# pangenome/impg

Hardware: AMD Instinct MI355X
Metric: projected ranges/sec, 1M-PAF 100k-BED -x depth 3; CPU coitrees baseline (higher is better)
Workload: dtype int32

## Files before the change

impg_amd/_lib.py:

```python
import ctypes as C
import os
import subprocess

import numpy as np

_HERE = os.path.dirname(os.path.abspath(__file__))
LIB_PATH = os.environ.get("IMPG_GPU_LIB") or os.path.join(_HERE, "libimpg_gpu.so")
CSRC = os.path.join(_HERE, "csrc")

IMPG_OK = 0
IMPG_E_INVALID, IMPG_E_HIP, IMPG_E_OOM, IMPG_E_IO, IMPG_E_UNSUPPORTED, IMPG_E_CANCELLED = -1, -2, -3, -4, -5, -6
STREAM_CB = C.CFUNCTYPE(C.c_int, C.c_void_p, C.c_void_p, C.c_size_t)
ORDER_COITREES, ORDER_SORTED = 0, 1
HIT_NONE = 0xFFFFFFFF

RECORD_DTYPE = np.dtype([("query_id", "<u4"), ("target_id", "<u4"), ("query_start", "<i4"), ("query_end", "<i4"),
                         ("target_start", "<i4"), ("target_end", "<i4"), ("cigar_off", "<u8"), ("cigar_len", "<u4"),
                         ("strand", "<u4")], align=True)
RANGE_DTYPE = np.dtype([("target_id", "<u4"), ("start", "<i4"), ("end", "<i4")])
INTERVAL_DTYPE = np.dtype([("query_id", "<u4"), ("q_first", "<i4"), ("q_last", "<i4"),
                           ("target_id", "<u4"), ("t_first", "<i4"), ("t_last", "<i4")])
assert RECORD_DTYPE.itemsize == 40 and RANGE_DTYPE.itemsize == 12
TP_RECORD_DTYPE = np.dtype([("query_id", "<u4"), ("target_id", "<u4"), ("query_start", "<i4"), ("query_end", "<i4"),
                            ("target_start", "<i4"), ("target_end", "<i4"), ("seg_off", "<u8"), ("n_segs", "<u4"),
# ... 96 lines not shown
    ("impg_gpu_query_batch_filtered", C.c_int, [_P, _P, C.c_size_t, C.POINTER(Params), _P, _P, C.POINTER(_P)]),
    ("impg_gpu_parse_subsequence", C.c_int, [C.c_char_p, C.c_char_p, C.c_size_t, C.POINTER(C.c_int32)]),
    ("impg_gpu_subset_keep", C.c_int, [C.c_char_p, C.c_size_t, _P, C.c_size_t, _P, C.POINTER(C.c_size_t)]),
    ("impg_gpu_query", C.c_int, [_P, C.c_uint32, C.c_int32, C.c_int32, C.POINTER(Params), C.POINTER(_P)]),
    ("impg_gpu_results_num_ranges", C.c_size_t, [_P]),
    ("impg_gpu_results_total", C.c_size_t, [_P]),
    ("impg_gpu_results_offsets", _P, [_P]),
    ("impg_gpu_results_intervals", _P, [_P]),
    ("impg_gpu_results_projected", C.c_uint64, [_P]),
    ("impg_gpu_results_cigar_offsets", _P, [_P]),
    ("impg_gpu_results_cigar_ops", _P, [_P]),
    ("impg_gpu_results_timing", None, [_P, C.POINTER(C.c_double), C.POINTER(C.c_double)]),
    ("impg_gpu_results_free", None, [_P]),
    ("impg_gpu_query_batch_stats", C.c_int, [_P, _P, C.c_size_t, C.POINTER(Params), _P, _P, C.POINTER(Stats)]),
    ("impg_gpu_query_batch_stats_dev", C.c_int, [_P, _P, C.c_size_t, C.POINTER(Params), _P, _P, C.POINTER(Stats)]),
    ("impg_gpu_query_batch_device", C.c_int, [_P, _P, C.c_size_t, C.c_int, C.POINTER(Params), C.c_int, C.POINTER(_P)]),
    ("impg_gpu_device_rows_num_parts", C.c_size_t, [_P]),
    ("impg_gpu_device_rows_part", C.c_int, [_P, C.c_size_t, C.POINTER(DevicePart)]),
    ("impg_gpu_device_rows_stats", None, [_P, C.POINTER(Stats)]),
    ("impg_gpu_device_rows_place_ms", C.c_float, [_P]),
    ("impg_gpu_device_rows_part_device", C.c_int, [_P, C.c_size_t, C.POINTER(C.c_int)]),
    ("impg_gpu_device_rows_batch_offset", C.c_int, [_P, C.POINTER(C.c_uint64), C.POINTER(C.c_uint64)]),
    ("impg_gpu_device_rows_check", C.c_int, [_P, _P, _P]),
    ("impg_gpu_device_rows_free", None, [_P]),
    ("impg_gpu_bed_merge", C.c_long, [_P, C.c_size_t, C.c_int32, C.c_int]),
    ("impg_gpu_results_bed", C.c_int, [_P, _P, _P, C.POINTER(Params), C.c_int32, C.POINTER(_P), C.POINTER(C.c_size_t)]),
    ("impg_gpu_query_batch_bed", C.c_int, [_P, _P, C.c_size_t, C.POINTER(Params), _P, C.c_int32, _P, C.POINTER(_P), C.POINTER(C.c_size_t),
                                           _P]),
    ("impg_gpu_query_batch_bed_fd", C.c_int, [_P, _P, C.c_size_t, C.POINTER(Params), _P, C.c_int32, _P, C.c_int, C.POINTER(C.c_uint64), _P]),
    ("impg_gpu_results_paf", C.c_int, [_P, _P, _P, C.POINTER(Params), C.c_int32, C.c_int, C.POINTER(_P), C.POINTER(C.c_size_t)]),
    ("impg_gpu_parse_cigar", C.c_long, [C.c_char_p, C.c_size_t, _P, C.c_size_t]),
    ("impg_gpu_parse_target_range", C.c_int, [C.c_char_p, C.c_char_p, C.c_size_t, C.POINTER(C.c_int32), C.POINTER(C.c_int32)]),
    ("impg_gpu_comm_unique_id", C.c_int, [_P, C.c_int]),
    ("impg_gpu_comm_create_rccl", C.c_int, [_P, C.c_int, C.c_int, C.c_int, C.c_int, C.POINTER(_P)]),
    ("impg_gpu_comm_create_host", C.c_int, [_P, C.c_int, C.c_int, C.c_int, C.c_int, C.POINTER(_P)]),
    ("impg_gpu_comm_destroy", None, [_P]),
    ("impg_gpu_comm_info", C.c_int, [_P, C.POINTER(C.c_int), C.POINTER(C.c_int), C.POINTER(C.c_int), C.POINTER(C.c_char_p)]),
    ("impg_gpu_comm_check", C.c_int, [_P, C.c_int]),
    ("impg_gpu_index_create_rank", C.c_int, [_P, C.c_size_t, _P, C.c_size_t, _P, C.c_uint32, _P, C.c_uint32, C.c_int, C.c_int,
                                             C.c_int, _P, C.POINTER(_P)]),
    ("impg_gpu_index_create_from_paf_rank", C.c_int, [C.POINTER(C.c_char_p), C.c_int, C.c_int, C.c_int, C.c_int, _P, C.POINTER(_P)]),
    ("impg_gpu_index_create_multi", C.c_int, [_P, C.c_size_t, _P, C.c_size_t, _P, C.c_uint32, _P, C.c_uint32, C.c_int, C.c_int,
                                              _P, C.c_int, C.c_int, C.POINTER(_P)]),
    ("impg_gpu_index_create_from_paf_multi", C.c_int, [C.POINTER(C.c_char_p), C.c_int, C.c_int, C.c_int, _P, C.c_int, C.c_int,
                                                       C.POINTER(_P)]),
    ("impg_gpu_shard_assign", C.c_int, [_P, C.c_uint32, C.c_uint32, _P]),
    ("impg_gpu_index_shard_info", C.c_int, [_P, C.POINTER(C.c_int), C.POINTER(C.c_int), C.POINTER(C.c_int), _P, C.c_size_t]),
    ("impg_gpu_index_hop_profile", C.c_int, [_P, _P, C.c_size_t, C.c_int, C.POINTER(C.c_size_t)]),
    ("impg_synth_paf", C.c_int, [C.c_uint64, C.c_size_t, C.c_uint32, C.c_int32, C.c_int32, C.c_uint32, _P, _P, C.c_size_t,
                                 C.POINTER(C.c_size_t)]),
    ("impg_synth_paf_text", C.c_int, [C.c_uint64, C.c_size_t, C.c_uint32, C.c_int32, C.c_int32, C.c_uint32, C.c_char_p]),
    ("impg_synth_skewed_paf_text", C.c_int, [C.c_uint64, C.c_size_t, C.c_uint32, C.c_int32, C.c_char_p, C.POINTER(C.c_uint64)]),
    ("impg_gpu_selftest_order_sort", C.c_int, [C.c_int, C.c_uint32, C.c_uint, C.c_uint64]),
    ("impg_synth_seq_name", C.c_int, [C.c_uint32, C.c_char_p, C.c_size_t]),
    ("impg_synth_bed", C.c_int, [C.c_uint64, C.c_size_t, C.c_uint32, C.c_int32, C.c_int32, _P]),
]

_LIB = None


def lib():
    global _LIB
    if _LIB is None:
        if not os.path.exists(LIB_PATH):
            raise RuntimeError("libimpg_gpu.so is not built: run `python -c 'import __graft_entry__ as g; g.build()'` "
                               "or `make -C impg_amd/csrc` (there is no CPU fallback)")
        L = C.CDLL(LIB_PATH)
        for name, res, args in SYMBOLS:
            f = getattr(L, name)
            f.restype = res
            f.argtypes = args
        _LIB = L
    return _LIB


def check(rc):
    if rc != IMPG_OK:
        raise ImpgGpuError(rc, lib().impg_gpu_last_error().decode(errors="replace"))


def free(ptr):
    C.CDLL(None).free(ptr)
```

impg_amd/csrc/capi.cpp:

```cpp
#include <sys/stat.h>
#include <unistd.h>

#include <atomic>
#include <cerrno>
#include <functional>
#include <thread>
#include <chrono>
#include <cmath>
#include <cstdlib>
#include <memory>
#include <new>

#include "engine.hpp"

namespace impg {
thread_local std::string g_error;
void set_error(const std::string &msg) { g_error = msg; }
void render_paf(const impg_gpu_results &res, const impg_gpu_index &ix, const char *const *range_names,
                const impg_gpu_params_t &p, int32_t merge_distance, bool bedpe, std::vector<std::string> &parts);
void render_bed(const impg_gpu_results &res, const impg_gpu_index &ix, const char *const *range_names,
                const impg_gpu_params_t &p, int32_t merge_distance, std::vector<std::string> &parts);
char *join_parts(std::vector<std::string> &parts, size_t *len);
}

// ... 1218 lines not shown
  std::vector<std::string> parts;
  render_paf(*res, *ix, range_names, *params, merge_distance, format == IMPG_OUT_BEDPE, parts);
  *text = join_parts(parts, len);
  return IMPG_OK;
  IMPG_CATCH
}

int impg_gpu_selftest_order_sort(int device, uint32_t n, unsigned end_bit, uint64_t seed) {
  IMPG_TRY
  if (end_bit < 1 || end_bit > 32) throw Error{IMPG_E_INVALID, "end_bit is 1 .. 32"};
  IMPG_HIP(hipSetDevice(device));
  std::vector<uint32_t> keys(n), perm(n);
  uint64_t x = seed * 0x9E3779B97F4A7C15ull + 0xD1B54A32D192ED03ull;
  const uint32_t mask = end_bit >= 32 ? 0xFFFFFFFFu : ((1u << end_bit) - 1u);
  for (uint32_t i = 0; i < n; i++) {
    x ^= x << 13; x ^= x >> 7; x ^= x << 17;
    keys[i] = (i % 7u == 3u && i) ? keys[i - 1] : (uint32_t)(x >> 20);
  }
  hipStream_t s;
  IMPG_HIP(hipStreamCreate(&s));
  DevBuf ka, kb, pa, pb, sc;
  const size_t nb = std::max<size_t>((size_t)n * 4, 256);
  ka.reserve(nb); kb.reserve(nb); pa.reserve(nb); pb.reserve(nb); sc.reserve(order_sort_scratch_bytes(n));
  IMPG_HIP(hipMemcpyAsync(ka.p, keys.data(), (size_t)n * 4, hipMemcpyHostToDevice, s));
  IMPG_HIP(hipMemsetAsync(pa.p, 0xA5, nb, s));
  launch_order_sort(ka.as<uint32_t>(), kb.as<uint32_t>(), pa.as<uint32_t>(), pb.as<uint32_t>(), n, end_bit, sc.p, s);
  IMPG_HIP(hipGetLastError());
  IMPG_HIP(hipMemcpyAsync(perm.data(), pa.p, (size_t)n * 4, hipMemcpyDeviceToHost, s));
  IMPG_HIP(hipStreamSynchronize(s));
  IMPG_HIP(hipStreamDestroy(s));
#ifdef IMPG_OS_CLOCKS
  {
    unsigned long long c[8];
    order_sort_clocks(c, false);
    fprintf(stderr, "[order sort clocks] n=%u bits=%u tiles x passes=%llu: per tile-pass zero+load %.0f rank %.0f bases %.0f lds %.0f out %.0f cycles\n", n, end_bit, c[7],
            (double)c[0] / c[7], (double)c[1] / c[7], (double)c[2] / c[7], (double)c[3] / c[7], (double)c[4] / c[7]);
    order_sort_clocks(nullptr, true);
  }
#endif
  std::vector<uint8_t> seen(n, 0);
  for (uint32_t k = 0; k < n; k++) {
    const uint32_t i = perm[k];
    if (i >= n || seen[i]) throw Error{IMPG_E_INVALID, "order sort: not a permutation at place " + std::to_string(k)};
    seen[i] = 1;
    if (k) {
      const uint32_t a = keys[perm[k - 1]] & mask, b = keys[i] & mask;
      if (a > b || (a == b && perm[k - 1] > i)) throw Error{IMPG_E_INVALID, "order sort: out of order at place " + std::to_string(k)};
    }
  }
  return IMPG_OK;
  IMPG_CATCH
}

}
```

impg_amd/csrc/engine.cpp:

```cpp
#include <cmath>
#include <cstdio>
#include <cstdlib>
#include <memory>

#include "engine.hpp"

namespace impg {

namespace {
inline unsigned bits_for(uint64_t n) {
  unsigned b = 0;
  while ((1ull << b) < n) b++;
  return b;
}
}

Engine::Engine(int device) {
  IMPG_HIP(hipSetDevice(device));
  IMPG_HIP(hipStreamCreateWithFlags(&stream, hipStreamNonBlocking));
  for (DevBuf *b : {&ord_offsets, &ord_rows}) b->pool = &level_pool;
  win_se.pool = &level_pool;
  counters.reserve(128);
  acc_slots.reserve(COUNT_BYTES);
  act_slots.reserve(COUNT_BYTES);
// ... 215 lines not shown
            n, wide ? "wide" : "wave", n_wg, members, slab / 1048576.0, a.dfs, a.max_depth, flags[1], st ? st->ms_total : -1.0f);
  ix.walk_last_members = members;
  if (flags[1]) { ix.walk_fallbacks++; return false; }
  ix.walk_launches++;
  if (st) st->levels = p.max_depth;
  return true;
}

Engine::~Engine() {
  if (small_in) (void)hipHostFree(small_in);
  if (small_out) (void)hipHostFree(small_out);
  for (auto e : ev_pool) (void)hipEventDestroy(e);
  if (h_counters) (void)hipHostFree(h_counters);
  if (h_slots) (void)hipHostFree(h_slots);
  if (stream) (void)hipStreamDestroy(stream);
}
hipEvent_t Engine::event() {
  if (ev_next == ev_pool.size()) {
    hipEvent_t e;
    IMPG_HIP(hipEventCreate(&e));
    ev_pool.push_back(e);
  }
  return ev_pool[ev_next++];
}

uint64_t Engine::read_counter(int k) {
  IMPG_HIP(hipMemcpyAsync(h_counters, counters.as<uint64_t>() + k, 8, hipMemcpyDeviceToHost, stream));
  IMPG_HIP(hipStreamSynchronize(stream));
  return h_counters[0];
}

uint64_t Engine::read_slots(DevBuf &b) {
  IMPG_HIP(hipMemcpyAsync(h_slots, b.p, COUNT_BYTES, hipMemcpyDeviceToHost, stream));
  IMPG_HIP(hipStreamSynchronize(stream));
  uint64_t t = 0;
  for (uint32_t k = 0; k < COUNT_SLOTS; k++) t += h_slots[k * COUNT_STRIDE];
  return t;
}

uint64_t Engine::scan(const uint32_t *in, uint32_t *out, uint32_t n) {
  if (n == 0) return 0;
  scan_tmp.reserve(scan_scratch_bytes(n));
  launch_exclusive_scan(in, out, n, scan_tmp.as<unsigned long long>(), counters.as<unsigned long long>() + 3, stream);
  IMPG_HIP(hipMemcpyAsync(h_counters, counters.as<uint64_t>() + 3, 24, hipMemcpyDeviceToHost, stream));
  IMPG_HIP(hipStreamSynchronize(stream));
  if (h_counters[2]) throw Error{IMPG_E_INVALID, "query range must satisfy start < end"};
  return h_counters[0];
}

void Engine::scan2(const uint32_t *in_a, uint32_t *out_a, const uint32_t *in_b, uint32_t *out_b, uint32_t n, uint64_t &total_a, uint64_t &total_b,
                   const uint32_t *d_extra, uint32_t *h_extra, uint32_t n_extra) {
  total_a = total_b = 0;
  if (n) {
    scan_tmp.reserve(scan_scratch_bytes(n));
    scan_tmp2.reserve(scan_scratch_bytes(n));
    launch_exclusive_scan(in_a, out_a, n, scan_tmp.as<unsigned long long>(), counters.as<unsigned long long>() + 12, stream);
    launch_exclusive_scan(in_b, out_b, n, scan_tmp2.as<unsigned long long>(), counters.as<unsigned long long>() + 13, stream);
    IMPG_HIP(hipMemcpyAsync(h_counters, counters.as<uint64_t>() + 12, 16, hipMemcpyDeviceToHost, stream));
  }
  if (n_extra) IMPG_HIP(hipMemcpyAsync(h_counters + 2, d_extra, (size_t)n_extra * 4, hipMemcpyDeviceToHost, stream));
  IMPG_HIP(hipStreamSynchronize(stream));
  if (n) { total_a = h_counters[0]; total_b = h_counters[1]; }
  if (n_extra) memcpy(h_extra, h_counters + 2, (size_t)n_extra * 4);
}

static HitArrays hit_arrays(LevelBufs &L, uint32_t n_pairs) {
  size_t b = std::max<size_t>((size_t)n_pairs * 4, 256);
  L.qid.reserve(L.qs_interleaved ? 2 * b : b); L.coords.reserve(4 * b);
  return HitArrays{L.qid.as<uint32_t>(), L.coords.as<int4>()};
}

const uint32_t *Engine::lookup_order(const DeviceIndexView &v, const FrontierRec *fr, uint32_t n_fr, const RecordBlocks *blocks) {
  if (!locality_min || (n_fr < locality_min && !blocks)) { keys_for = nullptr; return nullptr; }
  const size_t nb = (size_t)n_fr * 4;
  lo_key.reserve(nb); lo_key2.reserve(nb); lo_idx.reserve(nb); lo_perm.reserve(nb);
  unsigned hi_bit = std::max(1u, bits_for((uint32_t)std::min<size_t>(v.n_entries, 0xFFFFFFFFull)));
  unsigned block_shift = 0;
  if (blocks) {
    const unsigned bb = std::max(1u, bits_for(blocks->n_blocks));
    if (hi_bit + bb > 32) return nullptr;
    block_shift = hi_bit;
    hi_bit += bb;
  }
  if (!blocks && keys_for && keys_for == (const void *)fr && keys_n == n_fr) {
  } else
    launch_order_keys(v, fr, n_fr, lo_key.as<uint32_t>(), lo_idx.as<uint32_t>(), stream, blocks ? blocks->d_bounds : nullptr,
                      blocks ? blocks->n_blocks : 0u, block_shift);
  keys_for = nullptr;
  static const bool lib_sort = getenv("IMPG_LIB_SORT") && atoi(getenv("IMPG_LIB_SORT")) != 0;
  if (lib_sort) {
    const size_t tb = sort_u32_scratch_bytes(n_fr);
    sort_tmp.reserve(tb);
    launch_sort_u32(sort_tmp.p, tb, lo_key.as<uint32_t>(), lo_key2.as<uint32_t>(), lo_idx.as<uint32_t>(), lo_perm.as<uint32_t>(), n_fr,
                    stream, 0, hi_bit);
  } else {
    sort_tmp.reserve(order_sort_scratch_bytes(n_fr));
    launch_order_sort(lo_key.as<uint32_t>(), lo_key2.as<uint32_t>(), lo_perm.as<uint32_t>(), lo_idx.as<uint32_t>(), n_fr, hi_bit, sort_tmp.p, stream);
  }
  return lo_perm.as<uint32_t>();
}
void Engine::projection_offsets(const uint32_t *d_perm, uint32_t n_fr, const uint32_t *d_cnt, uint64_t P, const uint32_t *&d_offp,
                                ProjList &pl) {
  d_offp = nullptr;
  pl = ProjList{nullptr, nullptr, nullptr};
  if (!d_perm || !P) return;
  const size_t nb = (size_t)n_fr * 4;
  lo_cnt.reserve(nb); lo_off.reserve(nb); lo_offp.reserve(nb);
  const size_t pb = std::max<size_t>(P * 4, 256);
  slot_of.reserve(pb); proj_range.reserve(pb); proj_entry.reserve(pb);
  launch_gather_u32(d_cnt, d_perm, n_fr, lo_cnt.as<uint32_t>(), stream);
// ... 766 lines not shown
```

impg_amd/csrc/engine.hpp:

```cpp
#pragma once
#include <atomic>
#include <functional>
#include <memory>
#include <string>
#include <vector>

#include "kernels.hpp"

namespace impg {

struct LevelBufs {
  DevBuf frontier, pair_range, qid, coords;
  DevBuf sl_a, sl_n, sl_off, sl_rem, slice_pos, slice_pool;
  uint64_t slice_total = 0;
  uint32_t n_frontier = 0, n_pairs = 0;
  DevBuf slot_ref, lvbase, run_start;
  bool qs_interleaved = false;
  bool placed = false;
  LevelBufs() = default;
  explicit LevelBufs(BufPool *pool) {
    for (DevBuf *b : {&frontier, &pair_range, &qid, &coords, &sl_a, &sl_n, &sl_off, &sl_rem, &slice_pos, &slice_pool, &slot_ref, &lvbase, &run_start}) b->pool = pool;
  }
};
struct VisitedStore {
  DevBuf keys, off, len, ranges, qoff;
  uint32_t n_groups = 0;
  explicit VisitedStore(BufPool *pool) { keys.pool = off.pool = len.pool = ranges.pool = qoff.pool = pool; }
};

struct SplitBatch {};

struct HopResult {
  uint64_t pairs;
  bool all_dead;
};
struct Engine;
struct Expander {
  virtual ~Expander() {}
  virtual HopResult hop(Engine &home, const DeviceIndexView &v, const FrontierRec *fr, uint32_t n_fr, bool transitive,
                        LevelBufs &L, impg_gpu_stats_t *st, bool need_hits, bool need_rows, bool alive) = 0;
};

struct Engine {
  BufPool table_pool;
  BufPool level_pool;
  hipStream_t stream = nullptr;
  DevBuf counters;
  DevBuf acc_slots, act_slots;
  uint64_t *h_slots = nullptr;
  uint64_t read_slots(DevBuf &b);
  uint64_t *h_counters = nullptr;
  std::vector<hipEvent_t> ev_pool;
  size_t ev_next = 0;
  struct Timed { hipEvent_t a, b; int kind; };
  std::vector<Timed> timed;
  DevBuf big_list;
  DevBuf cnt, win, pair_off, pair_entry, scan_tmp, scan_tmp2, keys, skeys, vals, svals, sort_tmp, head, gid, gstart, glen, old_src,
      cap, pcap, poff, pieces, n_pieces, foff, frontier_a, frontier_b, self_scratch, ranges_dev, stat_count,
      stat_cksum, stage_off;
  LevelBufs level_scratch;
  std::vector<std::unique_ptr<VisitedStore>> tables;
  uint32_t table_queries = 0;
  void index_table(VisitedStore &t);
  uint64_t last_projected = 0;
  uint64_t pair_budget = 1ull << 28;
  uint32_t chunk_ranges = 0;
  bool split_ok = false;
  double min_identity = __builtin_nan("");
  bool store_cigar = false;
  bool multi = false;
  bool free_slot_order = false;
  bool free_slots_allowed = true;
  std::function<void()> on_kernels_done;
  bool regroup_pairs = true;
  bool fuse_allowed = true;
  bool fuse_final = false, fuse_need_ranges = false, fuse_range_places = false;
  bool last_range_places = false;
  bool keep_any_order = false;
  bool ordered_rows = false;
  DevBuf ord_acc, ord_offsets, ord_rows, ord_dest, ord_vpos, ord_cnt;
  uint64_t ord_total = 0;
  bool ord_offsets_done = false;
  uint32_t ord_n = 0;
  int32_t ord_min_len = -1;
  const FrontierRec *ord_self = nullptr;
  const impg_gpu_range_t *ord_ranges = nullptr;
  void ordered_level(const FrontierRec *fr, uint32_t n_fr, LevelBufs &L, bool counts_by_range, uint64_t P);
  void ordered_offsets();
  void ordered_finish(std::vector<std::unique_ptr<LevelBufs>> &levels);
  float ms_place = 0;
  DevBuf ent_work, ent_alloc;
  DevBuf win_se, tile_first;
  int filter_covered = 0;
  uint64_t covered_dropped = 0;
  DevBuf m_dest, m_qid, m_coords, m_pe, m_sa, m_sn, m_so, m_sr;
  DevBuf wide_n, wide_list;
  DevBuf lo_key, lo_key2, lo_idx, lo_perm, lo_cnt, lo_off, lo_offp, slot_of;
  uint32_t locality_min = 4096;
  const uint32_t *stage_perm = nullptr;
  uint32_t stage_n = 0;

  explicit Engine(int device);
  ~Engine();
  hipEvent_t event();
  uint64_t read_counter(int k);
  uint64_t scan(const uint32_t *in, uint32_t *out, uint32_t n);
  void scan2(const uint32_t *in_a, uint32_t *out_a, const uint32_t *in_b, uint32_t *out_b, uint32_t n, uint64_t &total_a, uint64_t &total_b,
             const uint32_t *d_extra = nullptr, uint32_t *h_extra = nullptr, uint32_t n_extra = 0);
  struct RecordBlocks { const uint32_t *d_bounds; uint32_t n_blocks; };
  const uint32_t *lookup_order(const DeviceIndexView &v, const FrontierRec *fr, uint32_t n_fr, const RecordBlocks *blocks = nullptr);
// ... 171 lines not shown
```

impg_amd/csrc/kernels.hip:

```cpp
#include <hip/hip_runtime.h>

#include <cstring>
#include <rocprim/device/device_radix_sort.hpp>

#include "impg_internal.hpp"
#include "kernels.hpp"

namespace impg {

__device__ __forceinline__ unsigned lane_id() { return threadIdx.x & 63u; }
__device__ __forceinline__ unsigned long long lanemask_lt() { return (1ull << lane_id()) - 1ull; }

template <int CTRL, int ROW_MASK>
__device__ __forceinline__ uint32_t dpp_or0(uint32_t x) {
  return (uint32_t)__builtin_amdgcn_update_dpp(0, (int)x, CTRL, ROW_MASK, 0xF, false);
}
__device__ __forceinline__ uint32_t wave_incl_scan(uint32_t x) {
  x += dpp_or0<0x111, 0xF>(x);
  x += dpp_or0<0x112, 0xF>(x);
  x += dpp_or0<0x114, 0xF>(x);
  x += dpp_or0<0x118, 0xF>(x);
  x += dpp_or0<0x142, 0xA>(x);
  x += dpp_or0<0x143, 0xC>(x);
  return x;
// ... 683 lines not shown
#pragma unroll
  for (uint32_t k = 0; k < SCAN_ITEMS; k++) {
    uint32_t i = base + k * SCAN_BLOCK + threadIdx.x;
    if (i < n) s += in[i];
  }
  uint32_t tot;
  block_excl_scan(s, &tot);
  if (threadIdx.x == 0) bsum[blockIdx.x] = tot;
}
__global__ __launch_bounds__(1024) void scan_of_sums(unsigned long long *bsum, uint32_t nb, unsigned long long *total) {
  __shared__ unsigned long long wsum[16];
  const uint32_t per = (nb + 1023u) / 1024u, a = min(nb, threadIdx.x * per), e = min(nb, a + per);
  unsigned long long mine = 0;
  for (uint32_t i = a; i < e; i++) mine += bsum[i];
  unsigned long long inc = mine;
#pragma unroll
  for (int d = 1; d < 64; d <<= 1) {
    const unsigned long long y = __shfl_up(inc, d);
    if ((int)lane_id() >= d) inc += y;
  }
  if (lane_id() == 63u) wsum[threadIdx.x >> 6] = inc;
  __syncthreads();
  unsigned long long base = 0;
  for (uint32_t k = 0; k < (threadIdx.x >> 6); k++) base += wsum[k];
  unsigned long long run = base + inc - mine;
  for (uint32_t i = a; i < e; i++) { const unsigned long long x = bsum[i]; bsum[i] = run; run += x; }
  if (threadIdx.x == 1023u) *total = run;
}
__global__ __launch_bounds__(256) void scan_apply(const uint32_t *__restrict__ in, uint32_t n,
                                                  const unsigned long long *__restrict__ bsum,
                                                  uint32_t *__restrict__ out) {
  uint32_t base = blockIdx.x * SCAN_TILE + threadIdx.x * SCAN_ITEMS;
  uint32_t x[SCAN_ITEMS];
  uint32_t s = 0;
#pragma unroll
  for (uint32_t k = 0; k < SCAN_ITEMS; k++) {
    uint32_t i = base + k;
    x[k] = i < n ? in[i] : 0;
    s += x[k];
  }
  uint32_t tot;
  uint32_t ex = block_excl_scan(s, &tot) + (uint32_t)bsum[blockIdx.x];
#pragma unroll
  for (uint32_t k = 0; k < SCAN_ITEMS; k++) {
    uint32_t i = base + k;
    if (i < n) out[i] = ex;
    ex += x[k];
  }
}

#ifndef IMPG_SCAN_LOOKBACK
#define IMPG_SCAN_LOOKBACK 1
#endif
constexpr uint32_t LB_ITEMS = 16, LB_BLOCK = 256, LB_TILE = LB_ITEMS * LB_BLOCK;
constexpr unsigned long long LB_FLAG_SUM = 1ull << 62, LB_FLAG_INCL = 2ull << 62, LB_VALUE = (1ull << 62) - 1ull;
__global__ __launch_bounds__(LB_BLOCK) void scan_lookback_kernel(const uint32_t *__restrict__ in, uint32_t *__restrict__ out, uint32_t n,
                                                                 unsigned long long *state, uint32_t n_tiles,
                                                                 unsigned long long *__restrict__ total) {
  __shared__ uint32_t s_tile;
  __shared__ unsigned long long s_prefix;
  if (threadIdx.x == 0) s_tile = atomicAdd(reinterpret_cast<uint32_t *>(state + n_tiles), 1u);
  __syncthreads();
  const uint32_t tile = s_tile;
  const uint32_t base = tile * LB_TILE + threadIdx.x * LB_ITEMS;
  uint32_t x[LB_ITEMS];
  if (base + LB_ITEMS <= n) {
    const uint4 *p = reinterpret_cast<const uint4 *>(in + base);
#pragma unroll
    for (uint32_t k = 0; k < LB_ITEMS / 4u; k++) {
      const uint4 v = p[k];
      x[4 * k] = v.x; x[4 * k + 1] = v.y; x[4 * k + 2] = v.z; x[4 * k + 3] = v.w;
    }
  } else {
#pragma unroll
    for (uint32_t k = 0; k < LB_ITEMS; k++) x[k] = base + k < n ? in[base + k] : 0u;
  }
  uint32_t mine = 0;
#pragma unroll
  for (uint32_t k = 0; k < LB_ITEMS; k++) mine += x[k];
  uint32_t tot;
  uint32_t ex = block_excl_scan(mine, &tot);
  if (tile == 0u) {
    if (threadIdx.x == 0) {
      __hip_atomic_store(state, LB_FLAG_INCL | (unsigned long long)tot, __ATOMIC_RELAXED, __HIP_MEMORY_SCOPE_AGENT);
      s_prefix = 0ull;
    }
  } else if (threadIdx.x < 64u) {
    if (threadIdx.x == 0)
      __hip_atomic_store(state + tile, LB_FLAG_SUM | (unsigned long long)tot, __ATOMIC_RELAXED, __HIP_MEMORY_SCOPE_AGENT);
    unsigned long long run = 0ull;
    int64_t j = (int64_t)tile - 1;
    for (;;) {
      const int64_t idx = j - (int64_t)threadIdx.x;
      unsigned long long w = LB_FLAG_INCL;
      unsigned long long incl, empty;
      uint32_t first;
      for (;;) {
        if (idx >= 0) w = __hip_atomic_load(state + idx, __ATOMIC_RELAXED, __HIP_MEMORY_SCOPE_AGENT);
        incl = __ballot((w >> 62) == 2ull);
        empty = __ballot((w >> 62) == 0ull);
        first = incl ? (uint32_t)__builtin_ctzll(incl) : 64u;
        const unsigned long long upto = first >= 63u ? ~0ull : (2ull << first) - 1ull;
        if (!(empty & upto)) break;
        __builtin_amdgcn_s_sleep(1);
      }
      unsigned long long v = threadIdx.x <= first ? (w & LB_VALUE) : 0ull;
#pragma unroll
      for (int o = 32; o > 0; o >>= 1) v += __shfl_xor(v, o);
      run += v;
      if (first < 64u) break;
      j -= 64;
    }
    if (threadIdx.x == 0) {
      s_prefix = run;
      __hip_atomic_store(state + tile, LB_FLAG_INCL | ((run + tot) & LB_VALUE), __ATOMIC_RELAXED, __HIP_MEMORY_SCOPE_AGENT);
    }
  }
  __syncthreads();
  const unsigned long long prefix = s_prefix;
  ex += (uint32_t)prefix;
  if (base + LB_ITEMS <= n) {
    uint4 *q = reinterpret_cast<uint4 *>(out + base);
#pragma unroll
    for (uint32_t k = 0; k < LB_ITEMS / 4u; k++) {
      uint4 v;
      v.x = ex; ex += x[4 * k];
      v.y = ex; ex += x[4 * k + 1];
      v.z = ex; ex += x[4 * k + 2];
      v.w = ex; ex += x[4 * k + 3];
      q[k] = v;
    }
  } else {
#pragma unroll
    for (uint32_t k = 0; k < LB_ITEMS; k++) {
      if (base + k < n) out[base + k] = ex;
      ex += x[k];
    }
  }
  if (tile == n_tiles - 1u && threadIdx.x == 0) *total = prefix + tot;
}

void launch_exclusive_scan(const uint32_t *d_in, uint32_t *d_out, uint32_t n, unsigned long long *d_bsum,
                           unsigned long long *d_total, hipStream_t s) {
  if (IMPG_SCAN_LOOKBACK && ((reinterpret_cast<uintptr_t>(d_in) | reinterpret_cast<uintptr_t>(d_out)) & 15u) == 0u) {
    const uint32_t nt = std::max<uint32_t>((n + LB_TILE - 1) / LB_TILE, 1u);
    IMPG_HIP(hipMemsetAsync(d_bsum, 0, ((size_t)nt + 1) * sizeof(unsigned long long), s));
    scan_lookback_kernel<<<nt, LB_BLOCK, 0, s>>>(d_in, d_out, n, d_bsum, nt, d_total);
    return;
  }
  uint32_t nb = (n + SCAN_TILE - 1) / SCAN_TILE;
  if (nb == 0) nb = 1;
  scan_block_sums<<<nb, SCAN_BLOCK, 0, s>>>(d_in, n, d_bsum);
  scan_of_sums<<<1, 1024, 0, s>>>(d_bsum, nb, d_total);
  scan_apply<<<nb, SCAN_BLOCK, 0, s>>>(d_in, n, d_bsum, d_out);
}
size_t scan_scratch_bytes(uint32_t n) { return ((size_t)(n + SCAN_TILE - 1) / SCAN_TILE + 2) * sizeof(unsigned long long); }

struct TileScan {
  bool found;
  bool any;
  int32_t pqs, pts, pqe, pte;
};
struct IdentScan {
  uint32_t rm, rx, rg;
  uint32_t fm, fx, fg;
  uint32_t lm, lx, lg;
  int32_t first_adj_m, first_adj_x;
  int32_t last_adj_m, last_adj_x;
  uint32_t first_oi, last_oi;
  int32_t first_off, last_rem;
};
constexpr int MODE_IDENT = 1, MODE_CIGAR = 2, MODE_WALK = 4;

struct PairCtx {
  int32_t ts, R0, R1, last_tp;
  bool swp, flip;
  uint32_t zt, zq;
  uint32_t m;
  uint32_t totT, totQ;
  const uint32_t *ops;
};

constexpr int PART_BOTH = 0, PART_FIRST = 1, PART_LAST = 2;
template <int MODE, int PART = PART_BOTH>
__device__ __forceinline__ void op_step(uint32_t op, const PairCtx &c, int32_t &T, int32_t &Qn, TileScan &s, IdentScan &id,
                                        uint32_t oi = 0) {
  constexpr bool IDENT = (MODE & MODE_IDENT) != 0;
  const bool valid = op != OP_PAD;
  const uint32_t code = op >> 29;
  const int32_t len = (int32_t)(op & OP_LEN_MASK);
  const int32_t td = code == c.zt ? 0 : len;
  const int32_t qa = code == c.zq ? 0 : len;
  const bool arm1 = td == 0;
  const bool qzero = qa == 0;
  const int32_t lim = qzero ? c.last_tp : c.R1;
  const int32_t os = max(T, c.R0);
  const int32_t e = T + td;
  const int32_t oe = min(e, lim);
  const int32_t slack = 1 - min(td, 1);
  const bool pass = valid & (T <= c.last_tp) & (os < oe + slack);
  const bool first = PART != PART_LAST && (pass & !s.found);
  if (IDENT) {
    const bool is_m = valid && (code == 0u || code == 4u), is_x = valid && code == 1u;
    const bool is_g = valid && (code == 2u || code == 3u);
    if (first) {
      id.fm = id.rm; id.fx = id.rx; id.fg = id.rg;
      const int32_t off = arm1 ? 0 : os - T;
// ... 4295 lines not shown
```

impg_amd/csrc/kernels.hpp:

```cpp
#pragma once
#include <hip/hip_runtime.h>

#include <cstdint>

#include "impg_internal.hpp"

namespace impg {

struct FrontierRec {
  uint32_t target_id;
  int32_t start, end;
  uint32_t qidx;
};

struct HitArrays {
  uint32_t *qid;
  int4 *c;
};

struct SliceArrays {
  uint32_t *a;
  uint32_t *n;
  int32_t *off;
  int32_t *rem;
// ... 38 lines not shown
  const uint8_t *vpos;
  int32_t min_output_length;
  uint32_t by_visit;
};
bool ordered_rows_by_visit();
struct WindowLists {
  const uint32_t *tile_first;
  const uint32_t *pair_off;
  const uint4 *win;
  const FrontierRec *se;
  const uint32_t *perm;
  uint32_t n_fr;
  uint32_t *range_out;
  uint32_t masks;
  uint32_t range_places;
  uint32_t *slice_work, *slice_alloc;
  uint32_t slice_cap;
  OrderedOut ord;
};
bool project_is_staged(const DeviceIndexView &v, uint64_t n_pairs, bool plain);
bool project_entry_major(const DeviceIndexView &v, uint64_t n_pairs, double min_identity);
uint32_t project_entry_blocks(uint32_t n_fr);
uint32_t project_entry_slice_cap(uint64_t n_pairs);
void launch_tile_first(const uint32_t *cnt, const uint32_t *pair_off, uint32_t n_fr, uint32_t *tile_first, hipStream_t s);
bool emit_by_lanes(const DeviceIndexView &v);
struct ProjList {
  uint32_t *slot, *range, *entry;
};
void launch_lookup_emit(const DeviceIndexView &v, const FrontierRec *fr, uint32_t n, bool transitive,
                        const uint32_t *pair_off, const uint4 *win, uint32_t *pair_range, uint32_t *pair_entry,
                        const uint32_t *perm, const uint32_t *offp, ProjList pl, const uint32_t *wide_n,
                        const uint32_t *wide_list, hipStream_t s, bool by_place = false, bool wide_only = false);
constexpr uint32_t ROUTE_WORLD_MAX = 1024;
void launch_route_keys(const FrontierRec *fr, uint32_t n, uint32_t world, const uint32_t *owner, uint32_t n_seq, uint32_t *key,
                       uint32_t *idx, unsigned long long *hist, hipStream_t s);
void launch_hits_pack(const FrontierRec *fr, const uint32_t *pair_range, uint32_t n_pairs, HitArrays h, const uint32_t *pair_entry,
                      const uint32_t *mrank, uint32_t words, void *out, hipStream_t s, const uint32_t *slice_n = nullptr);
void launch_hits_slice_n(const void *in, uint32_t n, uint32_t *cnt, hipStream_t s);
void launch_hits_unpack(const void *in, uint32_t n, uint32_t words, uint32_t n_front, const uint32_t *run_start, const uint32_t *off,
                        uint32_t *pair_range, HitArrays h, uint32_t *mslot, hipStream_t s, const uint32_t *slice_at = nullptr,
                        uint32_t *slice_pos = nullptr, uint32_t *slice_n = nullptr);
void launch_route_gather(const FrontierRec *fr, const uint32_t *perm, uint32_t n, FrontierRec *out, hipStream_t s);
void launch_route_gather_ranges(const FrontierRec *fr, const uint32_t *perm, uint32_t n, uint32_t range_base, FrontierRec *out, hipStream_t s);
void launch_partial_stats_add(const unsigned long long *in, uint32_t blocks, uint32_t n, unsigned long long *out, hipStream_t s);
void launch_frontier_gather(const FrontierRec *fr, const uint32_t *perm, uint32_t n, FrontierRec *out, hipStream_t s);
void launch_reorder_runs(const uint32_t *hits, uint32_t n, uint32_t words, uint32_t n_front, uint32_t *run_start,
                         uint32_t *run_len, uint32_t *err, hipStream_t s);
void launch_order_keys(const DeviceIndexView &v, const FrontierRec *fr, uint32_t n, uint32_t *key, uint32_t *idx, hipStream_t s,
                       const uint32_t *bounds = nullptr, uint32_t n_blocks = 0, uint32_t block_shift = 0);
void launch_scatter_u32(const uint32_t *in, const uint32_t *perm, uint32_t n, uint32_t *out, hipStream_t s);
void launch_exclusive_scan(const uint32_t *d_in, uint32_t *d_out, uint32_t n, unsigned long long *d_bsum,
                           unsigned long long *d_total, hipStream_t s);
size_t scan_scratch_bytes(uint32_t n);
enum ProjArm : int {
  PROJ_ARM_NONE = -1,
  PROJ_ARM_LANE = 0,
  PROJ_ARM_STAGED,
  PROJ_ARM_STAGED_ROWS,
  PROJ_ARM_ENTRIES_SLOTS,
  PROJ_ARM_ENTRIES_QS,
  PROJ_ARM_ENTRIES_ROWS,
  PROJ_ARM_ENTRIES_IDENT,
  PROJ_ARM_TP,
  PROJ_ARMS
};
static_assert(PROJ_ARMS == sizeof(impg_gpu_index::proj_stats) / sizeof(impg_gpu_index::proj_stats[0]), "one counter per arm");
int launch_project(const DeviceIndexView &v, const FrontierRec *fr, const uint32_t *pair_range,
                   const uint32_t *pair_entry, uint32_t n_pairs, bool transitive, HitArrays h,
                   unsigned long long *accepted, uint32_t *err_flag, double min_identity, const SliceArrays *slices,
                   ProjList pl, hipStream_t s, const uint32_t *n_pairs_dev = nullptr, bool regroup = false,
                   const WindowLists *wl = nullptr);
constexpr uint32_t SMALL_HEADER_BYTES = 64;
void launch_small_scan(const uint32_t *cnt, uint32_t n, uint32_t *off, uint32_t *total, hipStream_t s);
void launch_small_pack(const FrontierRec *fr, const uint32_t *pair_range, const uint32_t *n_pairs_dev, uint32_t pairs_bound, HitArrays h,
                       const uint32_t *err_flag, const unsigned long long *accepted, void *hdr, impg_gpu_interval_t *rows,
                       uint32_t *row_range, hipStream_t s);
void launch_slice_counts(HitArrays h, SliceArrays sl, uint32_t n_pairs, uint32_t *cnt, hipStream_t s);
void launch_slice_write(const DeviceIndexView &v, const uint32_t *pair_entry, HitArrays h, SliceArrays sl, uint32_t n_pairs,
                        const uint32_t *off, uint32_t *out, hipStream_t s);
void launch_hit_stats(const FrontierRec *fr, uint32_t n_fr, const uint32_t *pair_range, uint32_t n_pairs, HitArrays h,
                      int32_t min_output_length, bool skip_same_target, unsigned long long *rstat, unsigned long long *count,
                      unsigned long long *cksum, hipStream_t s, uint32_t stride = 1 );
void launch_sort5(const FrontierRec *fr, uint32_t n, const uint32_t *pair_off, uint32_t n_pairs, HitArrays h,
                  const uint32_t *pair_entry, const uint32_t *mrank, uint32_t *dest, hipStream_t s);
void launch_permute_slots(const uint32_t *dest, uint32_t n_pairs, HitArrays in, HitArrays out, const uint32_t *pe_in,
                          uint32_t *pe_out, SliceArrays sin, SliceArrays sout, hipStream_t s);
void launch_update_keys(const FrontierRec *fr, const uint32_t *pair_range, uint32_t n_pairs, HitArrays h,
                        unsigned long long *keys, unsigned long long *vals, unsigned long long *n_active, hipStream_t s);
size_t sort_pairs_scratch_bytes(uint32_t n);
void launch_sort_pairs(void *tmp, size_t tmp_bytes, const unsigned long long *kin, unsigned long long *kout,
                       const uint32_t *vin, uint32_t *vout, uint32_t n, unsigned end_bit, hipStream_t s);
uint32_t group_tiles(uint32_t n);
void launch_group_count(const unsigned long long *skeys, uint32_t n, uint32_t *tile_heads, hipStream_t s);
void launch_group_fill(const unsigned long long *skeys, uint32_t n, const uint32_t *tile_base, uint32_t *gstart, unsigned long long *gkey, hipStream_t s);
void launch_group_heads(const unsigned long long *skeys, uint32_t n, uint32_t *head, hipStream_t s);
void launch_group_scatter(const unsigned long long *skeys, uint32_t n, const uint32_t *head, const uint32_t *gid,
                          uint32_t *gstart, unsigned long long *gkey, hipStream_t s);
void launch_table_qoff(const unsigned long long *keys, uint32_t n_groups, uint32_t n_queries, uint32_t *qoff, hipStream_t s);
void launch_group_prepare(const VisitedTables &vt, const unsigned long long *gkey, const uint32_t *gstart,
                          uint32_t n_groups, uint32_t n_active, uint32_t *glen, const int2 **old_src,
                          uint32_t *cap, uint32_t *pcap, hipStream_t s);
void launch_visited_update(const unsigned long long *svals, const int32_t *seq_len,
                           const unsigned long long *gkey, const uint32_t *gstart, const uint32_t *glen,
                           const int2 *const *old_src, const uint32_t *noff, const uint32_t *poff,
                           uint32_t n_groups, int32_t min_transitive_len, int32_t mdbr, int2 *new_ranges,
                           uint32_t *new_len, int2 *pieces, uint32_t *n_pieces, const uint32_t *cap, const uint32_t *pcap,
// ... 130 lines not shown
```

include/impg_gpu.h:

```cpp
#ifndef IMPG_GPU_H
#define IMPG_GPU_H
#include <stddef.h>
#include <stdint.h>

#ifdef __cplusplus
extern "C" {
#endif

#define IMPG_OK 0
#define IMPG_E_INVALID (-1)
#define IMPG_E_HIP (-2)
#define IMPG_E_OOM (-3)
#define IMPG_E_IO (-4)
#define IMPG_E_UNSUPPORTED (-5)
#define IMPG_E_CANCELLED (-6)

typedef struct impg_gpu_index impg_gpu_index_t;
typedef struct impg_gpu_results impg_gpu_results_t;

typedef struct {
  uint32_t query_id, target_id;
  int32_t query_start, query_end;
  int32_t target_start, target_end;
  uint64_t cigar_off;
// ... 194 lines not shown
#define IMPG_OUT_BEDPE 1
int impg_gpu_results_paf(const impg_gpu_results_t *, const impg_gpu_index_t *,
                         const char *const *range_names, const impg_gpu_params_t *params,
                         int32_t merge_distance, int format, char **text, size_t *len);

long impg_gpu_parse_cigar(const char *cigar, size_t len, uint32_t *ops_out, size_t cap);
int impg_gpu_parse_subsequence(const char *seq_name, char *base_out, size_t base_cap, int32_t *start_offset);
int impg_gpu_parse_target_range(const char *s, char *name_out, size_t name_cap,
                                int32_t *start, int32_t *end);

typedef struct impg_gpu_comm impg_gpu_comm_t;
#define IMPG_COMM_ID_BYTES 128
int impg_gpu_comm_unique_id(uint8_t *ids, int lanes);
int impg_gpu_comm_create_rccl(const uint8_t *ids, int lanes, int rank, int world, int device, impg_gpu_comm_t **out);
typedef struct {
  void *ctx;
  int (*allgather_u64)(void *ctx, const uint64_t *mine, size_t k, uint64_t *all);
  int (*alltoallv)(void *ctx, const void *send, const uint64_t *send_off, const uint64_t *send_bytes, void *recv,
                   const uint64_t *recv_off, const uint64_t *recv_bytes);
} impg_gpu_host_transport_t;
int impg_gpu_comm_create_host(const impg_gpu_host_transport_t *transports , int lanes, int rank, int world,
                              int device, impg_gpu_comm_t **out);
void impg_gpu_comm_destroy(impg_gpu_comm_t *);
int impg_gpu_comm_info(const impg_gpu_comm_t *, int *rank, int *world, int *lanes, const char **kind );
int impg_gpu_comm_check(impg_gpu_comm_t *, int lane);
int impg_gpu_index_create_rank(const impg_gpu_record_t *records, size_t n_records, const uint32_t *cigar_ops, size_t n_ops,
                               const int64_t *seq_len, uint32_t n_seq, const uint64_t *file_first_record ,
                               uint32_t n_files, int bidirectional, int order_policy, int device, impg_gpu_comm_t *comm,
                               impg_gpu_index_t **out);
int impg_gpu_index_create_from_paf_rank(const char *const *paths, int n_paths, int bidirectional, int order_policy,
                                        int device, impg_gpu_comm_t *comm, impg_gpu_index_t **out);
int impg_gpu_index_create_multi(const impg_gpu_record_t *records, size_t n_records, const uint32_t *cigar_ops, size_t n_ops,
                                const int64_t *seq_len, uint32_t n_seq, const uint64_t *file_first_record ,
                                uint32_t n_files, int bidirectional, int order_policy, const int *devices, int n_dev,
                                int lanes, impg_gpu_index_t **out);
int impg_gpu_index_create_from_paf_multi(const char *const *paths, int n_paths, int bidirectional, int order_policy,
                                         const int *devices, int n_dev, int lanes, impg_gpu_index_t **out);
int impg_gpu_index_load_rank(const char *path, int device, impg_gpu_comm_t *comm, impg_gpu_index_t **out);
int impg_gpu_index_load_multi(const char *path, const int *devices, int n_dev, int lanes, impg_gpu_index_t **out);
int impg_gpu_shard_assign(const uint64_t *entries_per_target, uint32_t n_seq, uint32_t n_shards, uint32_t *owner_out);
int impg_gpu_index_shard_info(const impg_gpu_index_t *, int *rank, int *world, int *lanes, uint32_t *owner_out, size_t cap);
int impg_gpu_index_hop_profile(impg_gpu_index_t *, double *out, size_t cap, int reset, size_t *n_out);

int impg_synth_paf(uint64_t seed, size_t n_records, uint32_t n_seq, int32_t seq_len,
                   int32_t target_span, uint32_t n_blocks, impg_gpu_record_t *records,
                   uint32_t *ops, size_t ops_cap, size_t *n_ops_out);
int impg_synth_paf_text(uint64_t seed, size_t n_records, uint32_t n_seq, int32_t seq_len,
                        int32_t target_span, uint32_t n_blocks, const char *path);
int impg_synth_seq_name(uint32_t id, char *out, size_t cap);
int impg_synth_skewed_paf_text(uint64_t seed, size_t n_records, uint32_t n_seq, int32_t seq_len, const char *path, uint64_t *n_ops_out);
int impg_synth_bed(uint64_t seed, size_t n, uint32_t n_seq, int32_t seq_len, int32_t range_len,
                   impg_gpu_range_t *out);
int impg_gpu_selftest_order_sort(int device, uint32_t n, unsigned end_bit, uint64_t seed);

#ifdef __cplusplus
}
#endif
#endif
```

Baseline: 71.36 billion.

## Batch paired exclusive scans into one decoupled-lookback launch with coalesced tiles

```diff
diff --git a/impg_amd/_lib.py b/impg_amd/_lib.py
--- a/impg_amd/_lib.py
+++ b/impg_amd/_lib.py
@@ -172,6 +172,7 @@
     ("impg_synth_paf_text", C.c_int, [C.c_uint64, C.c_size_t, C.c_uint32, C.c_int32, C.c_int32, C.c_uint32, C.c_char_p]),
     ("impg_synth_skewed_paf_text", C.c_int, [C.c_uint64, C.c_size_t, C.c_uint32, C.c_int32, C.c_char_p, C.POINTER(C.c_uint64)]),
     ("impg_gpu_selftest_order_sort", C.c_int, [C.c_int, C.c_uint32, C.c_uint, C.c_uint64]),
+    ("impg_gpu_selftest_scan_batch", C.c_int, [C.c_int, C.POINTER(C.c_uint32), C.c_uint32, C.c_uint64]),
     ("impg_synth_seq_name", C.c_int, [C.c_uint32, C.c_char_p, C.c_size_t]),
     ("impg_synth_bed", C.c_int, [C.c_uint64, C.c_size_t, C.c_uint32, C.c_int32, C.c_int32, _P]),
 ]
diff --git a/impg_amd/csrc/capi.cpp b/impg_amd/csrc/capi.cpp
--- a/impg_amd/csrc/capi.cpp
+++ b/impg_amd/csrc/capi.cpp
@@ -1294,4 +1294,54 @@
   IMPG_CATCH
 }
 
-}
+int impg_gpu_selftest_scan_batch(int device, const uint32_t *lens, uint32_t count, uint64_t seed) {
+  IMPG_TRY
+  if (!lens || !count || count > SCAN_BATCH_MAX) throw Error{IMPG_E_INVALID, "a scan batch takes 1 .. 4 arrays"};
+  IMPG_HIP(hipSetDevice(device));
+  hipStream_t s;
+  IMPG_HIP(hipStreamCreate(&s));
+  constexpr uint32_t GUARD = 8;
+  std::vector<std::vector<uint32_t>> in(count), out(count);
+  std::vector<DevBuf> din(count), dout(count);
+  DevBuf sc, tot;
+  sc.reserve(std::max<size_t>(scan_batch_scratch_bytes(lens, count), 256));
+  tot.reserve(256);
+  IMPG_HIP(hipMemsetAsync(tot.p, 0xA5, 256, s));
+  std::vector<ScanJob> jobs(count);
+  uint64_t x = seed * 0x9E3779B97F4A7C15ull + 0xD1B54A32D192ED03ull;
+  for (uint32_t k = 0; k < count; k++) {
+    const uint32_t n = lens[k];
+    in[k].resize(n); out[k].resize((size_t)n + GUARD);
+    for (uint32_t i = 0; i < n; i++) {
+      x ^= x << 13; x ^= x >> 7; x ^= x << 17;
+      in[k][i] = i % 5u == 2u ? 0u : (uint32_t)(x >> 60);
+    }
+    din[k].reserve(std::max<size_t>((size_t)n * 4, 256));
+    dout[k].reserve(std::max<size_t>(((size_t)n + GUARD) * 4, 256));
+    if (n) IMPG_HIP(hipMemcpyAsync(din[k].p, in[k].data(), (size_t)n * 4, hipMemcpyHostToDevice, s));
+    IMPG_HIP(hipMemsetAsync(dout[k].p, 0xA5, ((size_t)n + GUARD) * 4, s));
+    jobs[k] = ScanJob{din[k].as<uint32_t>(), dout[k].as<uint32_t>(), n, tot.as<unsigned long long>() + k};
+  }
+  launch_exclusive_scan_batch(jobs.data(), count, sc.p, s);
+  IMPG_HIP(hipGetLastError());
+  unsigned long long totals[SCAN_BATCH_MAX];
+  for (uint32_t k = 0; k < count; k++)
+    IMPG_HIP(hipMemcpyAsync(out[k].data(), dout[k].p, out[k].size() * 4, hipMemcpyDeviceToHost, s));
+  IMPG_HIP(hipMemcpyAsync(totals, tot.p, sizeof totals, hipMemcpyDeviceToHost, s));
+  IMPG_HIP(hipStreamSynchronize(s));
+  IMPG_HIP(hipStreamDestroy(s));
+  for (uint32_t k = 0; k < count; k++) {
+    uint64_t run = 0;
+    for (uint32_t i = 0; i < lens[k]; i++) {
+      if (out[k][i] != (uint32_t)run) throw Error{IMPG_E_INVALID, "scan batch: array " + std::to_string(k) + " differs at " + std::to_string(i)};
+      run += in[k][i];
+    }
+    if (totals[k] != run) throw Error{IMPG_E_INVALID, "scan batch: total of array " + std::to_string(k) + " differs"};
+    for (uint32_t i = 0; i < GUARD; i++)
+      if (out[k][lens[k] + i] != 0xA5A5A5A5u) throw Error{IMPG_E_INVALID, "scan batch: array " + std::to_string(k) + " written past its end"};
+  }
+  return IMPG_OK;
+  IMPG_CATCH
+}
+
+}
diff --git a/impg_amd/csrc/engine.cpp b/impg_amd/csrc/engine.cpp
--- a/impg_amd/csrc/engine.cpp
+++ b/impg_amd/csrc/engine.cpp
@@ -291,10 +291,10 @@
                    const uint32_t *d_extra, uint32_t *h_extra, uint32_t n_extra) {
   total_a = total_b = 0;
   if (n) {
-    scan_tmp.reserve(scan_scratch_bytes(n));
-    scan_tmp2.reserve(scan_scratch_bytes(n));
-    launch_exclusive_scan(in_a, out_a, n, scan_tmp.as<unsigned long long>(), counters.as<unsigned long long>() + 12, stream);
-    launch_exclusive_scan(in_b, out_b, n, scan_tmp2.as<unsigned long long>(), counters.as<unsigned long long>() + 13, stream);
+    const uint32_t ns[2] = {n, n};
+    scan_tmp.reserve(scan_batch_scratch_bytes(ns, 2));
+    const ScanJob jobs[2] = {{in_a, out_a, n, counters.as<unsigned long long>() + 12}, {in_b, out_b, n, counters.as<unsigned long long>() + 13}};
+    launch_exclusive_scan_batch(jobs, 2, scan_tmp.p, stream);
     IMPG_HIP(hipMemcpyAsync(h_counters, counters.as<uint64_t>() + 12, 16, hipMemcpyDeviceToHost, stream));
   }
   if (n_extra) IMPG_HIP(hipMemcpyAsync(h_counters + 2, d_extra, (size_t)n_extra * 4, hipMemcpyDeviceToHost, stream));
diff --git a/impg_amd/csrc/engine.hpp b/impg_amd/csrc/engine.hpp
--- a/impg_amd/csrc/engine.hpp
+++ b/impg_amd/csrc/engine.hpp
@@ -55,7 +55,7 @@
   struct Timed { hipEvent_t a, b; int kind; };
   std::vector<Timed> timed;
   DevBuf big_list;
-  DevBuf cnt, win, pair_off, pair_entry, scan_tmp, scan_tmp2, keys, skeys, vals, svals, sort_tmp, head, gid, gstart, glen, old_src,
+  DevBuf cnt, win, pair_off, pair_entry, scan_tmp, keys, skeys, vals, svals, sort_tmp, head, gid, gstart, glen, old_src,
       cap, pcap, poff, pieces, n_pieces, foff, frontier_a, frontier_b, self_scratch, ranges_dev, stat_count,
       stat_cksum, stage_off;
   LevelBufs level_scratch;
diff --git a/impg_amd/csrc/kernels.hip b/impg_amd/csrc/kernels.hip
--- a/impg_amd/csrc/kernels.hip
+++ b/impg_amd/csrc/kernels.hip
@@ -759,34 +759,55 @@
 #ifndef IMPG_SCAN_LOOKBACK
 #define IMPG_SCAN_LOOKBACK 1
 #endif
-constexpr uint32_t LB_ITEMS = 16, LB_BLOCK = 256, LB_TILE = LB_ITEMS * LB_BLOCK;
+constexpr uint32_t LB_VECS = 16, LB_BLOCK = 256, LB_WAVES = LB_BLOCK / 64, LB_TILE = LB_VECS * 4 * LB_BLOCK;
+static_assert(LB_VECS * LB_WAVES == 64, "the (row, wave) totals are scanned by one wave");
+static_assert(LB_TILE >= SCAN_TILE, "scan_scratch_bytes is sized by the smaller tile");
 constexpr unsigned long long LB_FLAG_SUM = 1ull << 62, LB_FLAG_INCL = 2ull << 62, LB_VALUE = (1ull << 62) - 1ull;
-__global__ __launch_bounds__(LB_BLOCK) void scan_lookback_kernel(const uint32_t *__restrict__ in, uint32_t *__restrict__ out, uint32_t n,
-                                                                 unsigned long long *state, uint32_t n_tiles,
-                                                                 unsigned long long *__restrict__ total) {
+__global__ __launch_bounds__(LB_BLOCK) void scan_lookback_kernel(ScanBatch batch) {
   __shared__ uint32_t s_tile;
   __shared__ unsigned long long s_prefix;
+  __shared__ uint32_t s_part[LB_VECS * LB_WAVES + 1];
+  uint32_t which = 0;
+#pragma unroll
+  for (uint32_t k = 1; k < SCAN_BATCH_MAX; k++) which += k < batch.count && blockIdx.x >= batch.d[k].block0 ? 1u : 0u;
+  const ScanDesc &D = batch.d[which];
+  const uint32_t *__restrict__ in = D.in;
+  uint32_t *__restrict__ out = D.out;
+  unsigned long long *state = D.state;
+  const uint32_t n = D.n, n_tiles = D.n_tiles;
   if (threadIdx.x == 0) s_tile = atomicAdd(reinterpret_cast<uint32_t *>(state + n_tiles), 1u);
   __syncthreads();
   const uint32_t tile = s_tile;
-  const uint32_t base = tile * LB_TILE + threadIdx.x * LB_ITEMS;
-  uint32_t x[LB_ITEMS];
-  if (base + LB_ITEMS <= n) {
-    const uint4 *p = reinterpret_cast<const uint4 *>(in + base);
-#pragma unroll
-    for (uint32_t k = 0; k < LB_ITEMS / 4u; k++) {
-      const uint4 v = p[k];
-      x[4 * k] = v.x; x[4 * k + 1] = v.y; x[4 * k + 2] = v.z; x[4 * k + 3] = v.w;
-    }
-  } else {
-#pragma unroll
-    for (uint32_t k = 0; k < LB_ITEMS; k++) x[k] = base + k < n ? in[base + k] : 0u;
-  }
-  uint32_t mine = 0;
-#pragma unroll
-  for (uint32_t k = 0; k < LB_ITEMS; k++) mine += x[k];
-  uint32_t tot;
-  uint32_t ex = block_excl_scan(mine, &tot);
+  const uint64_t tbase = (uint64_t)tile * LB_TILE;
+  const bool full = tbase + LB_TILE <= n;
+  const uint32_t wv = threadIdx.x >> 6;
+  uint4 x[LB_VECS];
+  uint32_t sum[LB_VECS], inc[LB_VECS];
+#pragma unroll
+  for (uint32_t k = 0; k < LB_VECS; k++) {
+    const uint64_t i = tbase + (uint64_t)(k * LB_BLOCK + threadIdx.x) * 4u;
+    if (full || i + 4u <= n) x[k] = *reinterpret_cast<const uint4 *>(in + i);
+    else {
+      x[k].x = i < n ? in[i] : 0u;
+      x[k].y = i + 1u < n ? in[i + 1u] : 0u;
+      x[k].z = i + 2u < n ? in[i + 2u] : 0u;
+      x[k].w = 0u;
+    }
+  }
+#pragma unroll
+  for (uint32_t k = 0; k < LB_VECS; k++) {
+    sum[k] = x[k].x + x[k].y + x[k].z + x[k].w;
+    inc[k] = wave_incl_scan(sum[k]);
+    if (lane_id() == 63u) s_part[k * LB_WAVES + wv] = inc[k];
+  }
+  __syncthreads();
+  if (threadIdx.x < 64u) {
+    const uint32_t v = s_part[threadIdx.x], iv = wave_incl_scan(v);
+    s_part[threadIdx.x] = iv - v;
+    if (threadIdx.x == 63u) s_part[64] = iv;
+  }
+  __syncthreads();
+  const uint32_t tot = s_part[64];
   if (tile == 0u) {
     if (threadIdx.x == 0) {
       __hip_atomic_store(state, LB_FLAG_INCL | (unsigned long long)tot, __ATOMIC_RELAXED, __HIP_MEMORY_SCOPE_AGENT);
@@ -825,41 +846,69 @@
   }
   __syncthreads();
   const unsigned long long prefix = s_prefix;
-  ex += (uint32_t)prefix;
-  if (base + LB_ITEMS <= n) {
-    uint4 *q = reinterpret_cast<uint4 *>(out + base);
-#pragma unroll
-    for (uint32_t k = 0; k < LB_ITEMS / 4u; k++) {
-      uint4 v;
-      v.x = ex; ex += x[4 * k];
-      v.y = ex; ex += x[4 * k + 1];
-      v.z = ex; ex += x[4 * k + 2];
-      v.w = ex; ex += x[4 * k + 3];
-      q[k] = v;
-    }
-  } else {
-#pragma unroll
-    for (uint32_t k = 0; k < LB_ITEMS; k++) {
-      if (base + k < n) out[base + k] = ex;
-      ex += x[k];
-    }
-  }
-  if (tile == n_tiles - 1u && threadIdx.x == 0) *total = prefix + tot;
-}
-
-void launch_exclusive_scan(const uint32_t *d_in, uint32_t *d_out, uint32_t n, unsigned long long *d_bsum,
-                           unsigned long long *d_total, hipStream_t s) {
-  if (IMPG_SCAN_LOOKBACK && ((reinterpret_cast<uintptr_t>(d_in) | reinterpret_cast<uintptr_t>(d_out)) & 15u) == 0u) {
-    const uint32_t nt = std::max<uint32_t>((n + LB_TILE - 1) / LB_TILE, 1u);
-    IMPG_HIP(hipMemsetAsync(d_bsum, 0, ((size_t)nt + 1) * sizeof(unsigned long long), s));
-    scan_lookback_kernel<<<nt, LB_BLOCK, 0, s>>>(d_in, d_out, n, d_bsum, nt, d_total);
-    return;
-  }
+#pragma unroll
+  for (uint32_t k = 0; k < LB_VECS; k++) {
+    const uint64_t i = tbase + (uint64_t)(k * LB_BLOCK + threadIdx.x) * 4u;
+    uint32_t ex = (uint32_t)prefix + s_part[k * LB_WAVES + wv] + inc[k] - sum[k];
+    uint4 v;
+    v.x = ex; ex += x[k].x;
+    v.y = ex; ex += x[k].y;
+    v.z = ex; ex += x[k].z;
+    v.w = ex;
+    if (full || i + 4u <= n) *reinterpret_cast<uint4 *>(out + i) = v;
+    else {
+      if (i < n) out[i] = v.x;
+      if (i + 1u < n) out[i + 1u] = v.y;
+      if (i + 2u < n) out[i + 2u] = v.z;
+    }
+  }
+  if (tile == n_tiles - 1u && threadIdx.x == 0) *D.total = prefix + tot;
+}
+
+static void launch_scan_three_pass(const uint32_t *d_in, uint32_t *d_out, uint32_t n, unsigned long long *d_bsum,
+                                   unsigned long long *d_total, hipStream_t s) {
   uint32_t nb = (n + SCAN_TILE - 1) / SCAN_TILE;
   if (nb == 0) nb = 1;
   scan_block_sums<<<nb, SCAN_BLOCK, 0, s>>>(d_in, n, d_bsum);
   scan_of_sums<<<1, 1024, 0, s>>>(d_bsum, nb, d_total);
   scan_apply<<<nb, SCAN_BLOCK, 0, s>>>(d_in, n, d_bsum, d_out);
+}
+void launch_exclusive_scan_batch(const ScanJob *jobs, uint32_t count, void *scratch, hipStream_t s) {
+  if (!count || count > SCAN_BATCH_MAX) throw Error{IMPG_E_INVALID, "internal: a scan batch takes 1 .. SCAN_BATCH_MAX scans"};
+  bool lookback = IMPG_SCAN_LOOKBACK != 0;
+  for (uint32_t k = 0; k < count; k++)
+    if ((reinterpret_cast<uintptr_t>(jobs[k].in) | reinterpret_cast<uintptr_t>(jobs[k].out)) & 15u) lookback = false;
+  unsigned long long *state = static_cast<unsigned long long *>(scratch);
+  if (!lookback) {
+    for (uint32_t k = 0; k < count; k++) {
+      launch_scan_three_pass(jobs[k].in, jobs[k].out, jobs[k].n, state, jobs[k].total, s);
+      state += scan_scratch_bytes(jobs[k].n) / sizeof(unsigned long long);
+    }
+    return;
+  }
+  ScanBatch b;
+  memset(&b, 0, sizeof b);
+  b.count = count;
+  uint32_t blocks = 0;
+  size_t words = 0;
+  for (uint32_t k = 0; k < count; k++) {
+    const uint32_t nt = (uint32_t)std::max<uint64_t>(((uint64_t)jobs[k].n + LB_TILE - 1) / LB_TILE, 1u);
+    b.d[k] = ScanDesc{jobs[k].in, jobs[k].out, state + words, jobs[k].total, jobs[k].n, nt, blocks};
+    blocks += nt;
+    words += (size_t)nt + 1;
+  }
+  IMPG_HIP(hipMemsetAsync(state, 0, words * sizeof(unsigned long long), s));
+  scan_lookback_kernel<<<blocks, LB_BLOCK, 0, s>>>(b);
+}
+void launch_exclusive_scan(const uint32_t *d_in, uint32_t *d_out, uint32_t n, unsigned long long *d_bsum,
+                           unsigned long long *d_total, hipStream_t s) {
+  const ScanJob job{d_in, d_out, n, d_total};
+  launch_exclusive_scan_batch(&job, 1, d_bsum, s);
+}
+size_t scan_batch_scratch_bytes(const uint32_t *n, uint32_t count) {
+  size_t b = 0;
+  for (uint32_t k = 0; k < count; k++) b += scan_scratch_bytes(n[k]);
+  return b;
 }
 size_t scan_scratch_bytes(uint32_t n) { return ((size_t)(n + SCAN_TILE - 1) / SCAN_TILE + 2) * sizeof(unsigned long long); }
 
diff --git a/impg_amd/csrc/kernels.hpp b/impg_amd/csrc/kernels.hpp
--- a/impg_amd/csrc/kernels.hpp
+++ b/impg_amd/csrc/kernels.hpp
@@ -114,6 +114,14 @@
 void launch_exclusive_scan(const uint32_t *d_in, uint32_t *d_out, uint32_t n, unsigned long long *d_bsum,
                            unsigned long long *d_total, hipStream_t s);
 size_t scan_scratch_bytes(uint32_t n);
+constexpr uint32_t SCAN_BATCH_MAX = 4;
+struct ScanJob { const uint32_t *in; uint32_t *out; uint32_t n; unsigned long long *total; };
+struct ScanDesc {
+  const uint32_t *in; uint32_t *out; unsigned long long *state, *total; uint32_t n, n_tiles, block0;
+};
+struct ScanBatch { ScanDesc d[SCAN_BATCH_MAX]; uint32_t count; };
+void launch_exclusive_scan_batch(const ScanJob *jobs, uint32_t count, void *scratch, hipStream_t s);
+size_t scan_batch_scratch_bytes(const uint32_t *n, uint32_t count);
 enum ProjArm : int {
   PROJ_ARM_NONE = -1,
   PROJ_ARM_LANE = 0,
diff --git a/include/impg_gpu.h b/include/impg_gpu.h
--- a/include/impg_gpu.h
+++ b/include/impg_gpu.h
@@ -270,6 +270,7 @@
 int impg_synth_bed(uint64_t seed, size_t n, uint32_t n_seq, int32_t seq_len, int32_t range_len,
                    impg_gpu_range_t *out);
 int impg_gpu_selftest_order_sort(int device, uint32_t n, unsigned end_bit, uint64_t seed);
+int impg_gpu_selftest_scan_batch(int device, const uint32_t *lens, uint32_t count, uint64_t seed);
 
 #ifdef __cplusplus
 }
```

Result: faster. 72.17 billion (median of 6 runs) (+1.1%).
